# tpoisonooo/how-to-optimize-gemm

Measured on NVIDIA H100. Metric: SGEMM GFLOP/s (square N=4096 point of the 256..4096 sweep), higher is better.
Workload: dtype f16x2(scaled split-f32)

## Files before the change

### how-to-optimize-gemm_b200/csrc/capi.cu

```cuda
#include "../../include/b200gemm.h"

#include <cuda.h>
#include <cuda_runtime.h>
#include <stdio.h>
#include <stdlib.h>
#include <string.h>

#include <atomic>
#include <mutex>
#include <vector>

#include "gemm_ffma.cuh"
#include "gemm_generic.cuh"
#include "gemm_mxf4.cuh"
#include "gemm_tc.cuh"

using namespace b200;

namespace {

std::atomic<unsigned long long> g_launches{0};
int g_split_tail = 1;

struct KernelTimer {
  static constexpr int CAP = 1024;
  bool on = false;
  int n = 0;
  cudaEvent_t ev[CAP][2] = {};
  void begin(cudaStream_t st) {
    if (!on || n >= CAP) return;
    if (!ev[n][0]) { cudaEventCreate(&ev[n][0]); cudaEventCreate(&ev[n][1]); }
    cudaEventRecord(ev[n][0], st);
  }
  void end(cudaStream_t st) {
    if (!on || n >= CAP) return;
    cudaEventRecord(ev[n][1], st);
    n++;
  }
} g_ktimer;
std::atomic<int> g_default_f32_mode{-1};
thread_local const char* t_last_kernel = "none";
struct Schedule { int tiles = 0, split = 0, full_tiles = 0, ctas = 0; };
thread_local Schedule t_last_schedule;
int g_dbg_b_lbo = 0, g_dbg_b_sbo = 0;

struct Call {
  cudaStream_t st = nullptr;
  int acc = 0;
  int axpby = 0;
  float alpha = 1.f, beta = 0.f;
  const void* bias = nullptr;
  int act = -1;
  int sm_reserve = 0;
  bool epi() const { return act >= 0; }
};

constexpr int kFlagSlots = 16;
struct Scratch { void* p = nullptr; size_t bytes = 0; };
struct HostPipe {
  bool ready = false;
  cudaStream_t h2d = nullptr, comp = nullptr, d2h = nullptr;
  cudaEvent_t in[8] = {}, done[8] = {};
  cudaError_t init() {
    if (ready) return cudaSuccess;
    cudaError_t e;
    if ((e = cudaStreamCreateWithFlags(&h2d, cudaStreamNonBlocking)) != cudaSuccess) return e;
    if ((e = cudaStreamCreateWithFlags(&comp, cudaStreamNonBlocking)) != cudaSuccess) return e;
    if ((e = cudaStreamCreateWithFlags(&d2h, cudaStreamNonBlocking)) != cudaSuccess) return e;
    for (int i = 0; i < 8; i++) {
      if ((e = cudaEventCreateWithFlags(&in[i], cudaEventDisableTiming)) != cudaSuccess) return e;
      if ((e = cudaEventCreateWithFlags(&done[i], cudaEventDisableTiming)) != cudaSuccess) return e;
    }
    ready = true;
    return cudaSuccess;
  }
};
struct DevCtx {
  int ok = 0;
  int sms = 0;
  int dev = -1;
  int* flags = nullptr;
  std::mutex flag_mu;
  unsigned flag_slot = 0;
  struct FlagUser {
    cudaStream_t st = nullptr;
    cudaEvent_t ev = nullptr;
    bool used = false;
  } flag_user[kFlagSlots];
  std::mutex ws_mu;
  Scratch ws;
  cudaEvent_t ws_event = nullptr;
  cudaStream_t ws_stream = nullptr;
  bool ws_busy = false;
  struct MaxBuf {
    unsigned slot = 0;
    float* buf = nullptr;
    size_t cap = 0;
    int dirty[2] = {0, 0};
  } cmax, amax;
  cudaStream_t aux = nullptr;
  cudaEvent_t aux_fork = nullptr, aux_join = nullptr;
  std::mutex host_mu;
  Scratch scr[4];
  HostPipe pipe;
  std::vector<const void*> attr_done;
};
constexpr int kMaxDevices = 64;
DevCtx g_ctx[kMaxDevices];
std::mutex g_mu;

typedef CUresult (*EncodeTiledFn)(CUtensorMap*, CUtensorMapDataType, cuuint32_t, void*,
                                  const cuuint64_t*, const cuuint64_t*, const cuuint32_t*,
                                  const cuuint32_t*, CUtensorMapInterleave, CUtensorMapSwizzle,
                                  CUtensorMapL2promotion, CUtensorMapFloatOOBfill);
EncodeTiledFn g_encode = nullptr;

thread_local DevCtx* t_ctx = nullptr;
thread_local int t_bound_dev = -1;

int ensure_device() {
  int dev = -1;
  if (cudaGetDevice(&dev) != cudaSuccess || dev < 0 || dev >= kMaxDevices) { cudaGetLastError(); t_ctx = nullptr; return B200_ERR_NO_DEVICE; }
  if (t_bound_dev != dev) {
    if (cudaSetDevice(dev) != cudaSuccess) { cudaGetLastError(); t_ctx = nullptr; return B200_ERR_NO_DEVICE; }
    t_bound_dev = dev;
  }
  DevCtx* c = &g_ctx[dev];
  t_ctx = c;
  if (c->ok == 1) return 0;
  std::lock_guard<std::mutex> lk(g_mu);
  if (c->ok == 1) return 0;
  cudaDeviceProp prop;
  if (cudaGetDeviceProperties(&prop, dev) != cudaSuccess) { cudaGetLastError(); c->ok = -1; return B200_ERR_NO_DEVICE; }
  if (prop.major != 9) { c->ok = -1; return B200_ERR_NO_DEVICE; }
  if (!g_encode) {
    void* fn = nullptr;
    cudaDriverEntryPointQueryResult qres;
    if (cudaGetDriverEntryPoint("cuTensorMapEncodeTiled", &fn, cudaEnableDefault, &qres) != cudaSuccess ||
        qres != cudaDriverEntryPointSuccess || !fn) {
      cudaGetLastError();
      c->ok = -1;
      return B200_ERR_NO_DEVICE;
    }
    g_encode = reinterpret_cast<EncodeTiledFn>(fn);
  }
  if (!c->flags) {
    if (cudaMalloc(&c->flags, kFlagSlots * 1024 * sizeof(int)) != cudaSuccess ||
        cudaMemset(c->flags, 0, kFlagSlots * 1024 * sizeof(int)) != cudaSuccess) {
      cudaGetLastError(); c->flags = nullptr; c->ok = -1; return B200_ERR_NO_DEVICE;
    }
  }
  if (!c->ws_event && cudaEventCreateWithFlags(&c->ws_event, cudaEventDisableTiming) != cudaSuccess) {
    cudaGetLastError(); c->ok = -1; return B200_ERR_NO_DEVICE;
  }
  for (auto& u : c->flag_user)
    if (!u.ev && cudaEventCreateWithFlags(&u.ev, cudaEventDisableTiming) != cudaSuccess) {
      cudaGetLastError(); u.ev = nullptr; c->ok = -1; return B200_ERR_NO_DEVICE;
    }
  c->dev = dev;
  c->sms = prop.multiProcessorCount;
  c->ok = 1;
  return 0;
}

template <typename Kern>
int ensure_smem_attr(Kern kern, int bytes) {
  const void* key = reinterpret_cast<const void*>(kern);
  {
    std::lock_guard<std::mutex> lk(g_mu);
    for (const void* k : t_ctx->attr_done) if (k == key) return 0;
  }
  cudaError_t e = cudaFuncSetAttribute(kern, cudaFuncAttributeMaxDynamicSharedMemorySize, bytes);
  if (e != cudaSuccess) { cudaGetLastError(); return (int)e; }
  std::lock_guard<std::mutex> lk(g_mu);
  t_ctx->attr_done.push_back(key);
  return 0;
}

struct MapKey {
  const void* ptr; int dtype; unsigned long long d0, d1, ld_bytes; unsigned b0, b1; int swz; int dev;
  unsigned long long d2, d2_bytes;
  bool operator==(const MapKey& o) const {
    return ptr == o.ptr && dtype == o.dtype && d0 == o.d0 && d1 == o.d1 && ld_bytes == o.ld_bytes &&
           b0 == o.b0 && b1 == o.b1 && swz == o.swz && dev == o.dev && d2 == o.d2 && d2_bytes == o.d2_bytes;
  }
};
struct MapEntry { MapKey key; CUtensorMap map; };
std::vector<MapEntry> g_maps;
size_t g_map_next = 0;
constexpr size_t kMapCache = 64;

int get_map(CUtensorMap* out, const void* ptr, CUtensorMapDataType dt, int elem_bytes,
            unsigned long long inner, unsigned long long rows, unsigned long long ld_bytes,
            unsigned box_inner, unsigned box_rows, int swizzle ,
            unsigned long long entries = 0, unsigned long long entry_bytes = 0) {
  MapKey key{ptr, (int)dt, inner, rows, ld_bytes, box_inner, box_rows, swizzle, t_ctx->dev, entries, entry_bytes};
  std::lock_guard<std::mutex> lk(g_mu);
  for (auto& e : g_maps)
    if (e.key == key) { *out = e.map; return 0; }
  cuuint64_t dims[3] = {inner, rows, entries};
  cuuint64_t strides[2] = {ld_bytes, entry_bytes};
  cuuint32_t box[3] = {box_inner, box_rows, 1};
  cuuint32_t estr[3] = {1, 1, 1};
  CUtensorMap m;
  CUresult r = g_encode(&m, dt, entries ? 3 : 2, const_cast<void*>(ptr), dims, strides, box, estr,
                        CU_TENSOR_MAP_INTERLEAVE_NONE,
                        swizzle == 1 ? CU_TENSOR_MAP_SWIZZLE_128B
                        : swizzle == 2 ? CU_TENSOR_MAP_SWIZZLE_128B_ATOM_32B
                        : swizzle == 3 ? CU_TENSOR_MAP_SWIZZLE_64B : CU_TENSOR_MAP_SWIZZLE_NONE,
                        CU_TENSOR_MAP_L2_PROMOTION_L2_256B, CU_TENSOR_MAP_FLOAT_OOB_FILL_NONE);
  (void)elem_bytes;
  if (r != CUDA_SUCCESS) return B200_ERR_TENSORMAP;
  if (g_maps.size() < kMapCache) g_maps.push_back({key, m});
  else { g_maps[g_map_next] = {key, m}; g_map_next = (g_map_next + 1) % kMapCache; }
  *out = m;
  return 0;
}

inline bool aligned16(const void* p) { return (reinterpret_cast<uintptr_t>(p) & 15) == 0; }

int check_args(int m, int n, int k, const void* A, int lda, const void* B, int ldb, const void* C, int ldc,
               int op_a = B200_OP_N, int op_b = B200_OP_N) {
  if ((op_a != B200_OP_N && op_a != B200_OP_T) || (op_b != B200_OP_N && op_b != B200_OP_T)) return B200_ERR_BAD_ARG;
  if (m < 0 || n < 0 || k < 0) return B200_ERR_BAD_ARG;
  if (m == 0 || n == 0) return 1;
  if (!C || ldc < n) return B200_ERR_BAD_ARG;
  if (k > 0 && (!A || !B || lda < (op_a ? m : k) || ldb < (op_b ? k : n))) return B200_ERR_BAD_ARG;
  return 0;
}

int last_launch_status() {
  cudaError_t e = cudaPeekAtLastError();
  if (e != cudaSuccess) { cudaGetLastError(); return (int)e; }
  return 0;
}

int g_pdl = 1;
int g_prepass_fork = 1;
template <typename... KArgs, typename... Args>
cudaError_t launch_pdl(void (*kern)(KArgs...), dim3 grid, dim3 block, size_t smem, cudaStream_t st, int cluster, Args&&... args) {
  cudaLaunchConfig_t cfg = {};
  cfg.gridDim = grid; cfg.blockDim = block; cfg.dynamicSmemBytes = smem; cfg.stream = st;
  cudaLaunchAttribute at[2];
  int n = 0;
  if (cluster > 1) {
    at[n].id = cudaLaunchAttributeClusterDimension;
    at[n].val.clusterDim.x = cluster; at[n].val.clusterDim.y = 1; at[n].val.clusterDim.z = 1;
    n++;
  }
  if (g_pdl) {
    at[n].id = cudaLaunchAttributeProgrammaticStreamSerialization;
    at[n].val.programmaticStreamSerializationAllowed = 1;
    n++;
  }
  cfg.attrs = at; cfg.numAttrs = n;
  return cudaLaunchKernelEx(&cfg, kern, std::forward<Args>(args)...);
}

constexpr long long kMaxGridY = 65535;
inline unsigned grid_y(long long blocks) { return (unsigned)(blocks < kMaxGridY ? blocks : kMaxGridY); }

template <typename T>
int launch_zero(int m, int n, T* C, int ldc, cudaStream_t st) {
  dim3 grid((n + 255) / 256, m < 4096 ? m : 4096);
  fill_zero_kernel<T><<<grid, 256, 0, st>>>(m, n, C, ldc);
  g_launches++;
  t_last_kernel = "fill_zero";
  return last_launch_status();
}

template <typename InT, typename OutT>
int launch_generic(int op_a, int op_b, int m, int n, int k, const void* A, int lda, const void* B, int ldb, void* C,
                   int ldc, const char* name, const Call& c) {
  const long long mblocks = (m + 63LL) / 64;
  dim3 grid((n + 63) / 64, grid_y(mblocks));
  const long long a_rs = op_a ? 1 : lda, a_cs = op_a ? lda : 1, b_rs = op_b ? 1 : ldb, b_cs = op_b ? ldb : 1;
  auto kern = mblocks > kMaxGridY ? gemm_generic_kernel<InT, OutT, true> : gemm_generic_kernel<InT, OutT>;
  kern<<<grid, 256, 0, c.st>>>(m, n, k, static_cast<const InT*>(A), a_rs, a_cs, static_cast<const InT*>(B), b_rs, b_cs,
                               static_cast<OutT*>(C), ldc, c.acc, nullptr, nullptr, c.axpby, c.alpha, c.beta,
                               static_cast<const InT*>(c.bias), c.act);
  g_launches++;
  t_last_kernel = name;
  return last_launch_status();
}

int launch_generic_requant(int m, int n, int k, const int8_t* A, int lda, const int8_t* B, int ldb, int8_t* C,
                           int ldc, const float* scales, const float* bias, cudaStream_t st) {
  const long long mblocks = (m + 63LL) / 64;
  dim3 grid((n + 63) / 64, grid_y(mblocks));
  auto kern = mblocks > kMaxGridY ? gemm_generic_kernel<int8_t, int8_t, true> : gemm_generic_kernel<int8_t, int8_t>;
  kern<<<grid, 256, 0, st>>>(m, n, k, A, lda, 1, B, ldb, 1, C, ldc, 0, scales, bias, 0, 1.f, 0.f, nullptr, -1);
  g_launches++;
  t_last_kernel = "generic_s8_requant_64x64";
  return last_launch_status();
}

int take_flag_slot(cudaStream_t st, int** flags, DevCtx::FlagUser** user) {
  DevCtx* c = t_ctx;
  const unsigned slot = c->flag_slot++ % kFlagSlots;
  *flags = c->flags + slot * 1024;
  *user = nullptr;
  cudaStreamCaptureStatus cs = cudaStreamCaptureStatusNone;
  if (cudaStreamIsCapturing(st, &cs) != cudaSuccess) { cudaGetLastError(); cs = cudaStreamCaptureStatusActive; }
  DevCtx::FlagUser* u = &c->flag_user[slot];
  cudaError_t e;
  if (cs == cudaStreamCaptureStatusNone) {
    if (u->used && (u->st != st || st == cudaStreamPerThread) && (e = cudaStreamWaitEvent(st, u->ev, 0)) != cudaSuccess) {
      cudaGetLastError();
      return (int)e;
    }
    *user = u;
// ... 278 lines not shown
}

inline long long pitch16(int cols, int elem) { return (((long long)cols * elem + 15) & ~15LL) / elem; }
inline size_t round1024(size_t b) { return (b + 1023) & ~(size_t)1023; }
size_t kmajor_ws_bytes(int op_a, int op_b, int m, int n, int k, int elem) {
  const size_t b = op_b ? 0 : (size_t)n * pitch16(k, elem) * elem;
  const size_t a = op_a ? (size_t)m * pitch16(k, elem) * elem : 0;
  return a ? round1024(b) + a : b;
}

template <typename E>
int stage_kmajor(int op_a, int op_b, int m, int n, int k, const void*& A, long long& lda, const void*& B, long long& ldb,
                 uint8_t* ws, cudaStream_t st, bool copy_a = false, bool copy_b = false) {
  const long long kp = pitch16(k, sizeof(E));
  if (!op_b) {
    E* d = reinterpret_cast<E*>(ws);
    if (copy_b) {
      const cudaError_t e = cudaMemcpy2DAsync(d, kp * sizeof(E), B, ldb * sizeof(E), (size_t)k * sizeof(E), n,
                                              cudaMemcpyDeviceToDevice, st);
      if (e != cudaSuccess) { cudaGetLastError(); return (int)e; }
    } else if (int rc = launch_transpose<E>(static_cast<const E*>(B), ldb, k, n, d, kp, st)) {
      return rc;
    }
    B = d; ldb = kp;
  }
  if (op_a) {
    E* d = reinterpret_cast<E*>(ws + (op_b ? 0 : round1024((size_t)n * kp * sizeof(E))));
    if (copy_a) {
      const cudaError_t e = cudaMemcpy2DAsync(d, kp * sizeof(E), A, lda * sizeof(E), (size_t)k * sizeof(E), m,
                                              cudaMemcpyDeviceToDevice, st);
      if (e != cudaSuccess) { cudaGetLastError(); return (int)e; }
    } else if (int rc = launch_transpose<E>(static_cast<const E*>(A), lda, k, m, d, kp, st)) {
      return rc;
    }
    A = d; lda = kp;
  }
  return 0;
}

template <int KIND, int BN, int STAGES, typename OutT>
int launch_tc_kmajor(int op_a, int op_b, int m, int n, int k, const void* A, long long lda, const void* B, long long ldb,
                     void* C, int ldc, const char* name, const Call& c, const float* row_max = nullptr,
                     const float* col_max = nullptr) {
  if (!op_a && op_b) return launch_tc<KIND, BN, STAGES, OutT>(m, n, k, A, lda, m, 0, B, ldb, n, 0, C, ldc, name, c, 0, row_max, col_max);
  using E = typename std::conditional<KIND == KIND_TF32, float, uint8_t>::type;
  WsLease ws(kmajor_ws_bytes(op_a, op_b, m, n, k, sizeof(E)), c.st);
  if (ws.rc) return ws.rc;
  if (int rc = stage_kmajor<E>(op_a, op_b, m, n, k, A, lda, B, ldb, ws.base(), c.st)) return rc;
  return launch_tc<KIND, BN, STAGES, OutT>(m, n, k, A, lda, m, 0, B, ldb, n, 0, C, ldc, name, c, 0, row_max, col_max);
}

const char* const kNamesTf32[3] = {"tc_tf32_128x256", "tc_tf32_128x192", "tc_tf32_128x128"};
int tc_tf32(int op_a, int op_b, int m, int n, int k, const void* A, int lda, const void* B, int ldb, void* C, int ldc,
            const Call& c) {
  return with_width(m, n, [&](auto W) {
    using Wd = decltype(W);
    return launch_tc_kmajor<KIND_TF32, Wd::BN, Wd::STAGES, float>(op_a, op_b, m, n, k, A, lda, B, ldb, C, ldc,
                                                                kNamesTf32[Wd::idx], c);
  });
}
int tc_s8(int op_a, int op_b, int m, int n, int k, const void* A, int lda, const void* B, int ldb, void* C, int ldc,
          const Call& c) {
  return with_width<false>(m, n, [&](auto W) {
    using Wd = decltype(W);
    return launch_tc_kmajor<KIND_I8, Wd::BN, Wd::STAGES, int32_t>(op_a, op_b, m, n, k, A, lda, B, ldb, C, ldc,
                                                                Wd::BN == 256 ? "tc_s8_128x256" : "tc_s8_128x128", c);
  });
}
int tc_s8_requant(int m, int n, int k, const void* A, int lda, const void* B, int ldb, void* C, int ldc,
                  const float* scales, const float* bias, const Call& c) {
  return with_width<false>(m, n, [&](auto W) {
    using Wd = decltype(W);
    return launch_tc_kmajor<KIND_I8, Wd::BN, Wd::STAGES, s8_out>(
        B200_OP_N, B200_OP_N, m, n, k, A, lda, B, ldb, C, ldc,
        Wd::BN == 256 ? "tc_s8_requant_128x256" : "tc_s8_requant_128x128", c, scales, bias);
  });
}

inline long long plane_pitch(int cols) { return ((long long)cols + 7) & ~7LL; }
inline int b_plane_rows(int k) { return (k + 31) & ~31; }

template <int NP>
int launch_split(const SplitJob& ja, const SplitJob& jb, int jobs, cudaStream_t st) {
  const long long wide = jobs == 2 && jb.dld > ja.dld ? jb.dld : ja.dld;
  const int tall = jobs == 2 && jb.plane_rows > ja.plane_rows ? jb.plane_rows : ja.plane_rows;
  const int gx = (int)((wide + 2047) / 2048);
  int gy = (t_ctx->sms * 8 + jobs * gx - 1) / (jobs * gx);
  if (gy > (tall + 1) / 2) gy = (tall + 1) / 2;
  if (gy < 1) gy = 1;
  launch_pdl(split_planes_kernel<NP>, dim3(gx, gy, jobs), dim3(256), 0, st, 1, ja, jb);
  g_launches += 1;
  return last_launch_status();
}

struct PlaneGeom {
  int rows, cols, plane_rows;
  long long pitch;
  size_t bytes(int np) const { return (size_t)np * plane_rows * pitch * 2; }
};
inline PlaneGeom plane_geom(bool k_along_rows, int rows, int cols) {
  return PlaneGeom{rows, cols, k_along_rows ? b_plane_rows(rows) : rows, plane_pitch(cols)};
}
inline PlaneGeom geom_a(int op_a, int m, int k) { return op_a ? plane_geom(true, k, m) : plane_geom(false, m, k); }
inline PlaneGeom geom_b(int op_b, int k, int n) { return op_b ? plane_geom(false, n, k) : plane_geom(true, k, n); }

size_t split_ws_bytes(int np, int op_a, int op_b, int m, int n, int k, bool prepB = false) {
  const size_t a = round1024(geom_a(op_a, m, k).bytes(np));
  return prepB ? a : a + geom_b(op_b, k, n).bytes(np);
}

KernelNames kNamesBf16x3 = TC_NAMES("tc_bf16x3"), kNamesBf16x2 = TC_NAMES("tc_bf16x2"), kNamesF16x2 = TC_NAMES("tc_f16x2");

template <int NP>
int gemm_f32_split(int op_a, int op_b, int m, int n, int k, const float* A, int lda, const float* B, int ldb, float* C,
                   int ldc, const uint16_t* prepB, const Call& c) {
  const PlaneGeom ga = geom_a(op_a, m, k), gb = geom_b(op_b, k, n);
  WsLease ws(split_ws_bytes(NP, op_a, op_b, m, n, k, prepB != nullptr), c.st);
  if (ws.rc) return ws.rc;
  uint16_t* pA = reinterpret_cast<uint16_t*>(ws.base());
  const uint16_t* pB = prepB ? prepB : reinterpret_cast<uint16_t*>(ws.base() + round1024(ga.bytes(NP)));
  const SplitJob ja{A, lda, ga.rows, ga.cols, pA, ga.pitch, ga.plane_rows},
                 jb{B, ldb, gb.rows, gb.cols, const_cast<uint16_t*>(pB), gb.pitch, gb.plane_rows};
  if (int rc = launch_split<NP>(ja, jb, prepB ? 1 : 2, c.st)) return rc;
  using Prod = typename std::conditional<NP == 3, ProdX3, ProdX2>::type;
  return with_layout(op_a, op_b, [&](auto L) {
    using Lay = decltype(L);
    return launch_tc<KIND_F16, 128, NP == 3 ? 4 : 6, float, Prod, 64, Lay::AL, Lay::BL>(
        m, n, k, pA, ga.pitch, NP * ga.plane_rows, ga.plane_rows, pB, gb.pitch, NP * gb.plane_rows, gb.plane_rows, C, ldc,
        (NP == 3 ? kNamesBf16x3 : kNamesBf16x2)[Lay::idx][2], c, g_split_chunk_k[NP == 3 ? 0 : 1]);
  });
}

struct F16Operand {
  const uint16_t* planes;
  long long pitch;
  int plane_rows;
  const float* maxv;
};

int launch_f16_split_rows(const float* A, long long lda, int rows, int cols, float* rmax, uint16_t* planes,
                          long long pitch, int plane_rows, cudaStream_t st) {
  int blocks = (plane_rows + 7) / 8;
  const int cap = t_ctx->sms * 16;
  if (blocks > cap) blocks = cap;
  if (blocks < 1) blocks = 1;
  if (cols <= 1024) launch_pdl(split_f16_rows_kernel<4>, dim3(blocks), dim3(256), 0, st, 1, A, (long long)lda, rows, cols, rmax, planes, pitch, plane_rows);
  else if (cols <= 2048) launch_pdl(split_f16_rows_kernel<8>, dim3(blocks), dim3(256), 0, st, 1, A, (long long)lda, rows, cols, rmax, planes, pitch, plane_rows);
  else if (cols <= 4096) launch_pdl(split_f16_rows_kernel<16>, dim3(blocks), dim3(256), 0, st, 1, A, (long long)lda, rows, cols, rmax, planes, pitch, plane_rows);
  else launch_pdl(split_f16_rows_kernel<0>, dim3(blocks), dim3(256), 0, st, 1, A, (long long)lda, rows, cols, rmax, planes, pitch, plane_rows);
  g_launches++;
  return last_launch_status();
}

int launch_f16_split_cols(const float* B, long long ldb, int rows, int cols, float* cmax, uint16_t* planes,
                          long long pitch, int plane_rows, float* zero_buf, int zero_n, cudaStream_t st) {
  const cudaError_t e1 = launch_pdl(col_absmax_kernel, dim3((cols + 1023) / 1024, grid_y((rows + 15LL) / 16)), dim3(256), 0,
                                    st, 1, B, (long long)ldb, rows, cols, reinterpret_cast<unsigned int*>(cmax));
  const int gx = (int)((pitch + 2047) / 2048);
  int gy = (t_ctx->sms * 8 + gx - 1) / gx;
  if (gy > (plane_rows + 1) / 2) gy = (plane_rows + 1) / 2;
  if (gy < 1) gy = 1;
  if (zero_buf && zero_n > gx * 2048) {
    cudaMemsetAsync(zero_buf, 0, (size_t)zero_n * 4, st);
    zero_buf = nullptr;
  }
  const cudaError_t e2 = launch_pdl(split_f16_cols_kernel, dim3(gx, gy), dim3(256), 0, st, 1, B, (long long)ldb, rows, cols, (const float*)cmax, planes, pitch, plane_rows, zero_buf, zero_n);
  g_launches += 2;
  if (e1 != cudaSuccess || e2 != cudaSuccess) { cudaGetLastError(); return (int)(e1 != cudaSuccess ? e1 : e2); }
  return last_launch_status();
}

int gemm_f16x2_core(int op_a, int op_b, int m, int n, int k, const F16Operand& a, const F16Operand& b, float* C, int ldc,
                    const Call& c) {
  constexpr int NP = 2;
  return with_layout(op_a, op_b, [&](auto L) {
    using Lay = decltype(L);
    return launch_tc<KIND_FP16, 128, 6, float, ProdX2, 64, Lay::AL, Lay::BL>(
        m, n, k, a.planes, a.pitch, NP * a.plane_rows, a.plane_rows, b.planes, b.pitch, NP * b.plane_rows, b.plane_rows, C,
        ldc, kNamesF16x2[Lay::idx][2], c, g_split_chunk_k[2], a.maxv, b.maxv);
  });
}

int cmax_reserve(DevCtx::MaxBuf& mb, int n, float** cur, float** other, int* other_dirty) {
  if (mb.cap < (size_t)n) {
    size_t cap = mb.cap ? 2 * mb.cap : 16384;
    if (cap < (size_t)n) cap = (size_t)n;
    if (mb.buf) { cudaDeviceSynchronize(); cudaFree(mb.buf); }
    mb.buf = nullptr; mb.cap = 0;
    cudaError_t e = cudaMalloc(&mb.buf, 2 * cap * sizeof(float));
    if (e == cudaSuccess) e = cudaMemset(mb.buf, 0, 2 * cap * sizeof(float));
    if (e != cudaSuccess) { cudaGetLastError(); return (int)e; }
    mb.cap = cap;
    mb.dirty[0] = mb.dirty[1] = 0;
  }
  const unsigned slot = mb.slot++ & 1u;
  *cur = mb.buf + slot * mb.cap;
  *other = mb.buf + (slot ^ 1u) * mb.cap;
  *other_dirty = mb.dirty[slot ^ 1u];
  mb.dirty[slot ^ 1u] = 0;
  mb.dirty[slot] = n;
  return 0;
}

struct F16Ws {
  PlaneGeom ga, gb;
  size_t a_off, r_off, rb_off, total;
};
F16Ws f16x2_ws(int op_a, int op_b, int m, int n, int k, bool prepA, bool prepB) {
  F16Ws w{geom_a(op_a, m, k), geom_b(op_b, k, n)};
  w.a_off = round1024(prepA ? 0 : w.ga.bytes(2));
  w.r_off = round1024(w.a_off + (prepB ? 0 : w.gb.bytes(2)));
  const size_t ra = prepA || op_a ? 0 : (size_t)m * 4;
  w.rb_off = round1024(w.r_off + ra);
  w.total = prepB || !op_b ? w.r_off + ra : w.rb_off + (size_t)n * 4;
  return w;
}

int gemm_f32_split_f16(int op_a, int op_b, int m, int n, int k, const float* A, int lda, const float* B, int ldb, float* C,
                       int ldc, const F16Operand* prepA, const F16Operand* prepB, const Call& c) {
  if (prepA && prepB) return gemm_f16x2_core(B200_OP_N, B200_OP_N, m, n, k, *prepA, *prepB, C, ldc, c);
  const F16Ws w = f16x2_ws(op_a, op_b, m, n, k, prepA != nullptr, prepB != nullptr);
  const PlaneGeom &ga = w.ga, &gb = w.gb;
  WsLease ws(w.total, c.st);
  if (ws.rc) return ws.rc;
  uint8_t* base = ws.base();
  F16Operand oa, ob;
  DevCtx* dc = t_ctx;
  const bool fork = !prepA && !prepB && g_prepass_fork && (double)m * k + (double)k * n >= 4.0e6;
  cudaStream_t sb = c.st;
  if (fork) {
    if (!dc->aux) {
      if (cudaStreamCreateWithFlags(&dc->aux, cudaStreamNonBlocking) != cudaSuccess ||
          cudaEventCreateWithFlags(&dc->aux_fork, cudaEventDisableTiming) != cudaSuccess ||
          cudaEventCreateWithFlags(&dc->aux_join, cudaEventDisableTiming) != cudaSuccess) { cudaGetLastError(); return B200_ERR_NO_DEVICE; }
    }
    cudaEventRecord(dc->aux_fork, c.st);
    cudaStreamWaitEvent(dc->aux, dc->aux_fork, 0);
    sb = dc->aux;
  }
  if (prepB) ob = *prepB;
  else if (op_b) {
    uint16_t* pB = reinterpret_cast<uint16_t*>(base + w.a_off);
    float* bmax = reinterpret_cast<float*>(base + w.rb_off);
    if (int rc = launch_f16_split_rows(B, ldb, n, k, bmax, pB, gb.pitch, gb.plane_rows, sb)) return rc;
    ob = F16Operand{pB, gb.pitch, gb.plane_rows, bmax};
  } else {
    uint16_t* pB = reinterpret_cast<uint16_t*>(base + w.a_off);
    float *cmax, *other;
    int other_dirty;
    if (int rc = cmax_reserve(dc->cmax, n, &cmax, &other, &other_dirty)) return rc;
    if (int rc = launch_f16_split_cols(B, ldb, k, n, cmax, pB, gb.pitch, gb.plane_rows, other, other_dirty, sb)) return rc;
    ob = F16Operand{pB, gb.pitch, gb.plane_rows, cmax};
  }
  if (prepA) oa = *prepA;
  else if (op_a) {
    uint16_t* pA = reinterpret_cast<uint16_t*>(base);
    float *amax, *other;
    int other_dirty;
    if (int rc = cmax_reserve(dc->amax, m, &amax, &other, &other_dirty)) return rc;
    if (int rc = launch_f16_split_cols(A, lda, k, m, amax, pA, ga.pitch, ga.plane_rows, other, other_dirty, c.st)) return rc;
    oa = F16Operand{pA, ga.pitch, ga.plane_rows, amax};
  } else {
    uint16_t* pA = reinterpret_cast<uint16_t*>(base);
    float* rmax = reinterpret_cast<float*>(base + w.r_off);
    if (int rc = launch_f16_split_rows(A, lda, m, k, rmax, pA, ga.pitch, ga.plane_rows, c.st)) return rc;
    oa = F16Operand{pA, ga.pitch, ga.plane_rows, rmax};
  }
  if (fork) {
    cudaEventRecord(dc->aux_join, dc->aux);
    cudaStreamWaitEvent(c.st, dc->aux_join, 0);
  }
  return gemm_f16x2_core(op_a, op_b, m, n, k, oa, ob, C, ldc, c);
}

template <class Cfg, class Kern>
int launch_ffma(Kern kern, int ctas_per_sm, const char* name, int m, int n, int k, const float* A, int lda,
                const float* B, int ldb, float* C, int ldc, const Call& c) {
  CUtensorMap tmA, tmB;
  int rc = get_map(&tmA, A, CU_TENSOR_MAP_DATA_TYPE_FLOAT32, 4, k, m, (unsigned long long)lda * 4, Cfg::BK, Cfg::BM, 1);
  if (rc) return rc;
  rc = get_map(&tmB, B, CU_TENSOR_MAP_DATA_TYPE_FLOAT32, 4, n, k, (unsigned long long)ldb * 4, Cfg::BN, Cfg::BK, 0);
  if (rc) return rc;
  FfmaParams p;
  p.C = C; p.ldc = ldc; p.M = m; p.N = n; p.K = k;
  p.vec_ok = aligned16(C) && (ldc % 4) == 0;
  p.accumulate = c.acc;
  p.axpby = c.axpby; p.alpha = c.alpha; p.beta = c.beta;
  p.tiles_m = (m + Cfg::BM - 1) / Cfg::BM;
  p.tiles_n = (n + Cfg::BN - 1) / Cfg::BN;
  p.group_m = 8;
  const int tiles = p.tiles_m * p.tiles_n, slots = ctas_per_sm * t_ctx->sms;
  const int rem = tiles % slots;
  const bool halves = g_ffma_halves && rem > 0 && 2 * rem <= slots;
  p.full_tiles = halves ? tiles - rem : tiles;
  const int ctas = p.full_tiles + 2 * (tiles - p.full_tiles);
  if (int arc = ensure_smem_attr(kern, Cfg::SMEM_BYTES)) return arc;
  g_ktimer.begin(c.st);
  kern<<<ctas, Cfg::THREADS, Cfg::SMEM_BYTES, c.st>>>(tmA, tmB, p);
  g_ktimer.end(c.st);
  g_launches++;
  t_last_kernel = name;
  return last_launch_status();
}

size_t strict_ws_bytes(int op_a, int op_b, int m, int n, int k) {
  const size_t a = op_a ? (size_t)m * pitch16(k, 4) * 4 : 0, b = op_b ? (size_t)k * pitch16(n, 4) * 4 : 0;
  return a && b ? round1024(a) + b : a + b;
}
// ... 1265 lines not shown
```

### how-to-optimize-gemm_b200/csrc/gemm_tc.cuh

```cuda
#pragma once
#include <cuda_fp16.h>
#include <string.h>
#include <type_traits>

#include "ptx.cuh"
#include "wgmma.cuh"

namespace b200 {

enum Layout { LAYOUT_K = 0, LAYOUT_MN = 1 };

template <int KIND> struct KindTraits;
template <> struct KindTraits<KIND_F16>  { static constexpr int ELEM = 2; static constexpr int B_LAYOUT = LAYOUT_MN; };
template <> struct KindTraits<KIND_FP16> { static constexpr int ELEM = 2; static constexpr int B_LAYOUT = LAYOUT_MN; };
template <> struct KindTraits<KIND_TF32> { static constexpr int ELEM = 4; static constexpr int B_LAYOUT = LAYOUT_K; };
template <> struct KindTraits<KIND_I8>   { static constexpr int ELEM = 1; static constexpr int B_LAYOUT = LAYOUT_K; };
template <> struct KindTraits<KIND_E4M3> { static constexpr int ELEM = 1; static constexpr int B_LAYOUT = LAYOUT_K; };
template <> struct KindTraits<KIND_E4M3E5M2> { static constexpr int ELEM = 1; static constexpr int B_LAYOUT = LAYOUT_K; };
template <> struct KindTraits<KIND_E5M2E4M3> { static constexpr int ELEM = 1; static constexpr int B_LAYOUT = LAYOUT_K; };

struct ProdSingle {
  static constexpr int N = 1, NPA = 1, NPB = 1;
  __host__ __device__ static constexpr int ia(int) { return 0; }
  __host__ __device__ static constexpr int ib(int) { return 0; }
// ... 1505 lines not shown
      for (int c = lane * 8; c < dld; c += 256) {
        *reinterpret_cast<uint4*>(d1 + c) = make_uint4(0, 0, 0, 0);
        *reinterpret_cast<uint4*>(d2 + c) = make_uint4(0, 0, 0, 0);
      }
      continue;
    }
    const float* s = src + (long long)r * ld;
    float mx = 0.f;
    if constexpr (VPL > 0) {
      float x[VPL][8];
#pragma unroll
      for (int j = 0; j < VPL; j++) {
        const int c = (j * 32 + lane) * 8;
#pragma unroll
        for (int e = 0; e < 8; e++) x[j][e] = 0.f;
        if (c < cols) load8(s, c, cols, vec, x[j]);
#pragma unroll
        for (int e = 0; e < 8; e++) mx = fmaxf(mx, fabsf(x[j][e]));
      }
#pragma unroll
      for (int o = 16; o > 0; o >>= 1) mx = fmaxf(mx, __shfl_xor_sync(0xffffffffu, mx, o));
      if (lane == 0) rmax[r] = mx;
      const int ex = -pow2_exp(mx);
#pragma unroll
      for (int j = 0; j < VPL; j++) {
        const int c = (j * 32 + lane) * 8;
        if (c < dld) {
#pragma unroll
          for (int e = 0; e < 8; e++) x[j][e] = scale_pow2(x[j][e], ex);
          uint4 h1, h2;
          split_f16x8(x[j], h1, h2);
          *reinterpret_cast<uint4*>(d1 + c) = h1;
          *reinterpret_cast<uint4*>(d2 + c) = h2;
        }
      }
    } else {
      for (int c0 = lane * 8; c0 < cols; c0 += 1024) {
        float x[4][8];
#pragma unroll
        for (int u = 0; u < 4; u++) {
          const int c = c0 + u * 256;
#pragma unroll
          for (int e = 0; e < 8; e++) x[u][e] = 0.f;
          if (c < cols) load8(s, c, cols, vec, x[u]);
#pragma unroll
          for (int e = 0; e < 8; e++) mx = fmaxf(mx, fabsf(x[u][e]));
        }
      }
#pragma unroll
      for (int o = 16; o > 0; o >>= 1) mx = fmaxf(mx, __shfl_xor_sync(0xffffffffu, mx, o));
      if (lane == 0) rmax[r] = mx;
      const int ex = -pow2_exp(mx);
      for (int c0 = lane * 8; c0 < dld; c0 += 512) {
        float x[2][8];
#pragma unroll
        for (int u = 0; u < 2; u++) {
          const int c = c0 + u * 256;
#pragma unroll
          for (int e = 0; e < 8; e++) x[u][e] = 0.f;
          if (c < cols) load8(s, c, cols, vec, x[u]);
        }
#pragma unroll
        for (int u = 0; u < 2; u++) {
          const int c = c0 + u * 256;
          if (c < dld) {
#pragma unroll
            for (int e = 0; e < 8; e++) x[u][e] = scale_pow2(x[u][e], ex);
            uint4 h1, h2;
            split_f16x8(x[u], h1, h2);
            *reinterpret_cast<uint4*>(d1 + c) = h1;
            *reinterpret_cast<uint4*>(d2 + c) = h2;
          }
        }
      }
    }
  }
}

__global__ void __launch_bounds__(256) col_absmax_kernel(const float* __restrict__ src, long long ld, int rows,
                                                         int cols, unsigned int* __restrict__ out) {
  constexpr int ROWS = 16;
  griddep_launch();
  griddep_wait();
  const int c = blockIdx.x * 1024 + threadIdx.x * 4;
  if (c >= cols) return;
  const int rblocks = (int)(((long long)rows + ROWS - 1) / ROWS);
  const bool vec = (ld & 3) == 0 && (reinterpret_cast<uintptr_t>(src) & 15) == 0 && c + 4 <= cols;
  float4 mx = make_float4(0.f, 0.f, 0.f, 0.f);
  for (int rb = blockIdx.y; rb < rblocks; rb += gridDim.y) {
    const int r0 = rb * ROWS, r1 = min(r0 + ROWS, rows);
    if (vec) {
#pragma unroll 16
      for (int r = r0; r < r1; r++) {
        const float4 v = __ldg(reinterpret_cast<const float4*>(src + (long long)r * ld + c));
        mx.x = fmaxf(mx.x, fabsf(v.x)); mx.y = fmaxf(mx.y, fabsf(v.y));
        mx.z = fmaxf(mx.z, fabsf(v.z)); mx.w = fmaxf(mx.w, fabsf(v.w));
      }
    } else {
      for (int r = r0; r < r1; r++) {
        const float* s = src + (long long)r * ld + c;
        mx.x = fmaxf(mx.x, fabsf(s[0]));
        if (c + 1 < cols) mx.y = fmaxf(mx.y, fabsf(s[1]));
        if (c + 2 < cols) mx.z = fmaxf(mx.z, fabsf(s[2]));
        if (c + 3 < cols) mx.w = fmaxf(mx.w, fabsf(s[3]));
      }
    }
  }
  const float m4[4] = {mx.x, mx.y, mx.z, mx.w};
#pragma unroll
  for (int e = 0; e < 4; e++)
    if (c + e < cols && __float_as_uint(m4[e]) > __ldcg(out + c + e)) atomicMax(out + c + e, __float_as_uint(m4[e]));
}

__global__ void __launch_bounds__(256) split_f16_cols_kernel(const float* __restrict__ src, long long ld, int rows,
                                                             int cols, const float* __restrict__ cmax,
                                                             uint16_t* __restrict__ dst, long long dld, int plane_rows,
                                                             float* __restrict__ zero_buf, int zero_n) {
  griddep_launch();
  griddep_wait();
  const int c = (int)(blockIdx.x * 256 + threadIdx.x) * 8;
  if (blockIdx.y == 0 && zero_buf != nullptr) {
#pragma unroll
    for (int e = 0; e < 8; e++)
      if (c + e < zero_n) zero_buf[c + e] = 0.f;
  }
  if (c >= dld) return;
  const bool vec = (ld & 3) == 0 && (reinterpret_cast<uintptr_t>(src) & 15) == 0;
  int ex[8];
#pragma unroll
  for (int e = 0; e < 8; e++) ex[e] = c + e < cols ? -pow2_exp(__ldg(cmax + c + e)) : 0;
  for (int r0 = blockIdx.y * 2; r0 < plane_rows; r0 += gridDim.y * 2) {
    float x[2][8];
#pragma unroll
    for (int u = 0; u < 2; u++) {
      const int r = r0 + u;
#pragma unroll
      for (int e = 0; e < 8; e++) x[u][e] = 0.f;
      if (r < rows) load8(src + (long long)r * ld, c, cols, vec, x[u]);
    }
#pragma unroll
    for (int u = 0; u < 2; u++) {
      const int r = r0 + u;
      if (r >= plane_rows) break;
#pragma unroll
      for (int e = 0; e < 8; e++) x[u][e] = scale_pow2(x[u][e], ex[e]);
      uint4 h1, h2;
      split_f16x8(x[u], h1, h2);
      *reinterpret_cast<uint4*>(dst + (long long)r * dld + c) = h1;
      *reinterpret_cast<uint4*>(dst + ((long long)plane_rows + r) * dld + c) = h2;
    }
  }
}

}
```

### how-to-optimize-gemm_b200/csrc/ptx.cuh

```cuda
#pragma once
#include <cuda.h>
#include <cuda_runtime.h>
#include <math.h>
#include <stdint.h>

namespace b200 {

__device__ __forceinline__ uint32_t smem_u32(const void* p) {
  return static_cast<uint32_t>(__cvta_generic_to_shared(p));
}

__device__ __forceinline__ void mbar_init(uint32_t bar, uint32_t count) {
  asm volatile("mbarrier.init.shared::cta.b64 [%0], %1;" ::"r"(bar), "r"(count) : "memory");
}
__device__ __forceinline__ void fence_barrier_init() {
  asm volatile("fence.mbarrier_init.release.cluster;" ::: "memory");
}
__device__ __forceinline__ void fence_proxy_async() {
  asm volatile("fence.proxy.async.shared::cta;" ::: "memory");
}
__device__ __forceinline__ void mbar_arrive_expect_tx(uint32_t bar, uint32_t bytes) {
  asm volatile("mbarrier.arrive.expect_tx.shared::cta.b64 _, [%0], %1;" ::"r"(bar), "r"(bytes)
               : "memory");
}
__device__ __forceinline__ void mbar_arrive(uint32_t bar) {
  asm volatile("mbarrier.arrive.shared::cta.b64 _, [%0];" ::"r"(bar) : "memory");
}
__device__ __forceinline__ bool mbar_try_wait(uint32_t bar, uint32_t parity) {
  uint32_t ok;
  asm volatile(
      "{\n\t.reg .pred p;\n\t"
      "mbarrier.try_wait.parity.shared::cta.b64 p, [%1], %2;\n\t"
      "selp.u32 %0, 1, 0, p;\n\t}"
      : "=r"(ok)
      : "r"(bar), "r"(parity)
      : "memory");
  return ok != 0;
}
__device__ __forceinline__ void mbar_wait(uint32_t bar, uint32_t parity) {
  if (mbar_try_wait(bar, parity)) return;
  const long long t0 = clock64();
  while (!mbar_try_wait(bar, parity)) {
    if (clock64() - t0 > 4000000000LL) { asm volatile("trap;"); }
  }
}

__device__ __forceinline__ void tma_prefetch_desc(const CUtensorMap* m) {
  asm volatile("prefetch.tensormap [%0];" ::"l"(reinterpret_cast<uint64_t>(m)) : "memory");
}
__device__ __forceinline__ void tma_load_2d(uint32_t dst_smem, const CUtensorMap* m, uint32_t bar,
                                            int c0, int c1) {
  asm volatile(
      "cp.async.bulk.tensor.2d.shared::cluster.global.tile.mbarrier::complete_tx::bytes "
      "[%0], [%1, {%3, %4}], [%2];"
      ::"r"(dst_smem), "l"(reinterpret_cast<uint64_t>(m)), "r"(bar), "r"(c0), "r"(c1)
      : "memory");
}
__device__ __forceinline__ void tma_load_3d(uint32_t dst_smem, const CUtensorMap* m, uint32_t bar,
                                            int c0, int c1, int c2) {
  asm volatile(
      "cp.async.bulk.tensor.3d.shared::cluster.global.tile.mbarrier::complete_tx::bytes "
      "[%0], [%1, {%3, %4, %5}], [%2];"
      ::"r"(dst_smem), "l"(reinterpret_cast<uint64_t>(m)), "r"(bar), "r"(c0), "r"(c1), "r"(c2)
      : "memory");
}
__device__ __forceinline__ void tma_load_2d_hint(uint32_t dst_smem, const CUtensorMap* m,
                                                 uint32_t bar, int c0, int c1, uint64_t policy) {
  asm volatile(
      "cp.async.bulk.tensor.2d.shared::cluster.global.tile.mbarrier::complete_tx::bytes"
      ".L2::cache_hint [%0], [%1, {%3, %4}], [%2], %5;"
      ::"r"(dst_smem), "l"(reinterpret_cast<uint64_t>(m)), "r"(bar), "r"(c0), "r"(c1), "l"(policy)
      : "memory");
}

enum MmaKind { KIND_F16 = 0 , KIND_TF32 = 1, KIND_I8 = 2, KIND_FP16 = 3 ,
               KIND_E4M3 = 4 , KIND_E4M3E5M2 = 5 , KIND_E5M2E4M3 = 6  };
enum Swz { SWZ_128B = 1, SWZ_64B = 2 };

__device__ __forceinline__ uint64_t make_sdesc(uint32_t smem_addr, uint32_t lbo_bytes, uint32_t sbo_bytes, uint32_t swz) {
  uint64_t d = 0;
  d |= (uint64_t)((smem_addr & 0x3FFFF) >> 4);
  d |= (uint64_t)((lbo_bytes >> 4) & 0x3FFF) << 16;
  d |= (uint64_t)((sbo_bytes >> 4) & 0x3FFF) << 32;
  d |= (uint64_t)swz << 62;
  return d;
}

__device__ __forceinline__ int32_t requant_s8(int32_t acc, float scale, float bias, bool has_bias) {
  float f = __fmul_rn(__int2float_rn(acc), scale);
  if (has_bias) f = __fadd_rn(f, bias);
  const float g = fminf(fmaxf(f, -200.0f), 200.0f);
  const float magic = 12582912.0f;
  float r = __fadd_rn(__fadd_rn(g, magic), -magic);
  if (fabsf(__fadd_rn(g, -r)) == 0.5f && fabsf(r) < fabsf(g)) r = __fadd_rn(r, copysignf(1.0f, g));
  r = fminf(fmaxf(r, -128.0f), 127.0f);
  const int32_t q = __float_as_int(__fadd_rn(r, magic)) - 0x4B400000;
  return f != f ? 0 : q;
}

enum EpiAct { ACT_NONE = 0, ACT_RELU = 1, ACT_GELU = 2, ACT_GELU_TANH = 3 };
template <int ACT>
__device__ __forceinline__ float epi_act(float t) {
  if constexpr (ACT == ACT_RELU) {
    return t < 0.f ? 0.f : t;
  } else if constexpr (ACT == ACT_GELU) {
    const float g = __fmul_rn(__fmul_rn(0.5f, t), erfcf(__fmul_rn(-0.707106781186547524f, t)));
    return t == -INFINITY ? -0.f : g;
  } else if constexpr (ACT == ACT_GELU_TANH) {
    const float u = __fmul_rn(0.797884560802865356f, __fmaf_rn(__fmul_rn(0.044715f, t), __fmul_rn(t, t), t));
    const float g = __fmul_rn(__fmul_rn(0.5f, t), __fadd_rn(1.f, tanhf(u)));
    return t == -INFINITY ? -0.f : g;
  } else {
    return t;
  }
}

template <int N> __device__ __forceinline__ void setmaxnreg_inc() { asm volatile("setmaxnreg.inc.sync.aligned.u32 %0;" ::"n"(N)); }
template <int N> __device__ __forceinline__ void setmaxnreg_dec() { asm volatile("setmaxnreg.dec.sync.aligned.u32 %0;" ::"n"(N)); }

__device__ __forceinline__ void griddep_launch() { asm volatile("griddepcontrol.launch_dependents;" ::: "memory"); }
__device__ __forceinline__ void griddep_wait() { asm volatile("griddepcontrol.wait;" ::: "memory"); }

__device__ __forceinline__ bool elect_one() {
  uint32_t pred;
  asm volatile("{\n\t.reg .pred p;\n\telect.sync _|p, 0xffffffff;\n\tselp.b32 %0, 1, 0, p;\n\t}" : "=r"(pred));
  return pred != 0;
}

constexpr int kMaxGroups = 1024;

__device__ __forceinline__ void group_table(const int* __restrict__ offs, int groups, int total_m, int rows, int* end,
                                            int* block) {
  for (int i = threadIdx.x; i < groups; i += blockDim.x) end[i + 1] = offs[i];
  __syncthreads();
  if (threadIdx.x < 32) {
    const int lane = threadIdx.x;
    int run_end = 0, run_blocks = 0;
    for (int base = 0; base < groups; base += 32) {
      const int g = base + lane;
      int e = max(g < groups ? end[g + 1] : 0, run_end);
#pragma unroll
      for (int d = 1; d < 32; d <<= 1) {
        const int o = __shfl_up_sync(0xffffffffu, e, d);
        if (lane >= d) e = max(e, o);
      }
      e = min(e, total_m);
      int prev = __shfl_up_sync(0xffffffffu, e, 1);
      if (lane == 0) prev = run_end;
      int b = (e - prev) / rows + ((e - prev) % rows != 0);
#pragma unroll
      for (int d = 1; d < 32; d <<= 1) {
        const int o = __shfl_up_sync(0xffffffffu, b, d);
        if (lane >= d) b += o;
      }
      if (g < groups) { end[g + 1] = e; block[g + 1] = run_blocks + b; }
      run_end = __shfl_sync(0xffffffffu, e, 31);
      run_blocks += __shfl_sync(0xffffffffu, b, 31);
    }
    if (lane == 0) { end[0] = 0; block[0] = 0; }
  }
  __syncthreads();
}

__device__ __forceinline__ int group_of(const int* block, int groups, int q) {
  int lo = 0, hi = groups - 1;
  while (lo < hi) {
    const int mid = (lo + hi + 1) >> 1;
    if (block[mid] <= q) lo = mid;
    else hi = mid - 1;
  }
  return lo;
}

}
```

Baseline: 187,800.

## Fuse column absmax and f16 split of B into one cluster strip kernel

Replaces the two-kernel path for B (column absmax pass, then split pass) with one kernel launched in 8-CTA clusters. Each cluster owns a 32-column strip and each CTA stages its share of rows in shared memory via cp.async. The CTAs reduce the per-column max across the cluster through distributed shared memory, then scale and split from shared memory. This reads B from global memory once instead of twice and saves a launch, at the cost of heavy shared memory use, cluster barriers and a size-gated fallback.

```diff
diff --git a/how-to-optimize-gemm_b200/csrc/capi.cu b/how-to-optimize-gemm_b200/csrc/capi.cu
--- a/how-to-optimize-gemm_b200/csrc/capi.cu
+++ b/how-to-optimize-gemm_b200/csrc/capi.cu
@@ -99,6 +99,7 @@
     int dirty[2] = {0, 0};
   } cmax, amax;
   cudaStream_t aux = nullptr;
+  int strip_rows = 0;
   cudaEvent_t aux_fork = nullptr, aux_join = nullptr;
   std::mutex host_mu;
   Scratch scr[4];
@@ -157,6 +158,9 @@
     if (!u.ev && cudaEventCreateWithFlags(&u.ev, cudaEventDisableTiming) != cudaSuccess) {
       cudaGetLastError(); u.ev = nullptr; c->ok = -1; return B200_ERR_NO_DEVICE;
     }
+  cudaFuncAttributes fa;
+  if (cudaFuncGetAttributes(&fa, split_f16_strip_kernel) != cudaSuccess) { cudaGetLastError(); c->ok = -1; return B200_ERR_NO_DEVICE; }
+  c->strip_rows = (int)((prop.sharedMemPerBlockOptin - fa.sharedSizeBytes) / (kStripW * sizeof(float)));
   c->dev = dev;
   c->sms = prop.multiProcessorCount;
   c->ok = 1;
@@ -741,8 +745,24 @@
   return last_launch_status();
 }
 
+constexpr int kStripCluster = 8, kStripWave = 3;
 int launch_f16_split_cols(const float* B, long long ldb, int rows, int cols, float* cmax, uint16_t* planes,
                           long long pitch, int plane_rows, float* zero_buf, int zero_n, cudaStream_t st) {
+  const int rp = (plane_rows + kStripCluster - 1) / kStripCluster;
+  const long long strips = (pitch + kStripW - 1) / kStripW;
+  if (rp <= t_ctx->strip_rows && strips * kStripCluster >= (long long)kStripWave * t_ctx->sms) {
+    if (int arc = ensure_smem_attr(split_f16_strip_kernel, t_ctx->strip_rows * kStripW * (int)sizeof(float))) return arc;
+    const cudaError_t e = launch_pdl(split_f16_strip_kernel, dim3((unsigned)(strips * kStripCluster)), dim3(256),
+                                     (size_t)rp * kStripW * sizeof(float), st, kStripCluster, B, (long long)ldb, rows,
+                                     cols, cmax, planes, pitch, plane_rows, rp, zero_buf, zero_n);
+    g_launches++;
+    if (e != cudaSuccess) {
+      cudaGetLastError();
+      if (zero_buf) cudaMemsetAsync(zero_buf, 0, (size_t)zero_n * 4, st);
+      return (int)e;
+    }
+    return last_launch_status();
+  }
   const cudaError_t e1 = launch_pdl(col_absmax_kernel, dim3((cols + 1023) / 1024, grid_y((rows + 15LL) / 16)), dim3(256), 0,
                                     st, 1, B, (long long)ldb, rows, cols, reinterpret_cast<unsigned int*>(cmax));
   const int gx = (int)((pitch + 2047) / 2048);
diff --git a/how-to-optimize-gemm_b200/csrc/gemm_tc.cuh b/how-to-optimize-gemm_b200/csrc/gemm_tc.cuh
--- a/how-to-optimize-gemm_b200/csrc/gemm_tc.cuh
+++ b/how-to-optimize-gemm_b200/csrc/gemm_tc.cuh
@@ -1681,4 +1681,92 @@
   }
 }
 
-}
+constexpr int kStripW = 32;
+__global__ void __launch_bounds__(256) split_f16_strip_kernel(const float* __restrict__ src, long long ld, int rows,
+                                                              int cols, float* __restrict__ cmax,
+                                                              uint16_t* __restrict__ dst, long long dld, int plane_rows,
+                                                              int rp, float* __restrict__ zero_buf, int zero_n) {
+  extern __shared__ __align__(16) float strip[];
+  __shared__ float red[8][kStripW];
+  __shared__ float part[kStripW], full[kStripW];
+  griddep_launch();
+  griddep_wait();
+  const int t = threadIdx.x;
+  if (zero_buf != nullptr)
+    for (long long i = (long long)blockIdx.x * 256 + t; i < zero_n; i += (long long)gridDim.x * 256) zero_buf[i] = 0.f;
+  const uint32_t rank = cluster_ctarank(), ncta = cluster_nctarank();
+  const int c0 = (int)(blockIdx.x / ncta) * kStripW;
+  const int r0 = (int)rank * rp;
+  const int np = max(min(r0 + rp, plane_rows) - r0, 0);
+  const int nl = max(min(r0 + rp, rows) - r0, 0);
+  {
+    const bool vec = (ld & 3) == 0 && (reinterpret_cast<uintptr_t>(src) & 15) == 0;
+    const int q = t & 7, c = c0 + 4 * q;
+    const int valid = min(max(cols - c, 0), 4);
+    for (int r = t >> 3; r < nl; r += 32) {
+      const float* s = src + (long long)(r0 + r) * ld + c;
+      const uint32_t d = smem_u32(strip + r * kStripW + 4 * q);
+      if (vec) {
+        asm volatile("cp.async.cg.shared.global [%0], [%1], 16, %2;" ::"r"(d), "l"(valid ? s : src), "r"(valid * 4) : "memory");
+      } else {
+#pragma unroll
+        for (int e = 0; e < 4; e++)
+          asm volatile("cp.async.ca.shared.global [%0], [%1], 4, %2;" ::"r"(d + 4 * e), "l"(e < valid ? s + e : src),
+                       "r"(e < valid ? 4 : 0) : "memory");
+      }
+    }
+    asm volatile("cp.async.wait_all;" ::: "memory");
+    __syncthreads();
+  }
+  {
+    const int j = t & (kStripW - 1), g = t >> 5;
+    float m = 0.f;
+#pragma unroll 8
+    for (int r = g; r < nl; r += 8) m = fmaxf(m, fabsf(strip[r * kStripW + j]));
+    red[g][j] = m;
+    __syncthreads();
+    if (t < kStripW) {
+#pragma unroll
+      for (int k = 1; k < 8; k++) m = fmaxf(m, red[k][t]);
+      part[t] = m;
+    }
+  }
+  cluster_arrive();
+  cluster_wait();
+  if (t < kStripW) {
+    float m = 0.f;
+    for (uint32_t k = 0; k < ncta; k++) m = fmaxf(m, ld_shared_cluster(&part[t], k));
+    full[t] = m;
+    if (rank == 0 && c0 + t < cols) cmax[c0 + t] = m;
+  }
+  cluster_arrive();
+  __syncthreads();
+  const int q = t & 3, c = c0 + 8 * q;
+  if (c < dld) {
+    int ex[8];
+#pragma unroll
+    for (int e = 0; e < 8; e++) ex[e] = c + e < cols ? -pow2_exp(full[8 * q + e]) : 0;
+    for (int r = t >> 2; r < np; r += 64) {
+      float x[8];
+      if (r < nl) {
+        const float4 v0 = *reinterpret_cast<const float4*>(strip + r * kStripW + 8 * q);
+        const float4 v1 = *reinterpret_cast<const float4*>(strip + r * kStripW + 8 * q + 4);
+        x[0] = v0.x; x[1] = v0.y; x[2] = v0.z; x[3] = v0.w;
+        x[4] = v1.x; x[5] = v1.y; x[6] = v1.z; x[7] = v1.w;
+      } else {
+#pragma unroll
+        for (int e = 0; e < 8; e++) x[e] = 0.f;
+      }
+#pragma unroll
+      for (int e = 0; e < 8; e++) x[e] = scale_pow2(x[e], ex[e]);
+      uint4 h1, h2;
+      split_f16x8(x, h1, h2);
+      const long long pr = r0 + r;
+      *reinterpret_cast<uint4*>(dst + pr * dld + c) = h1;
+      *reinterpret_cast<uint4*>(dst + ((long long)plane_rows + pr) * dld + c) = h2;
+    }
+  }
+  cluster_wait();
+}
+
+}
diff --git a/how-to-optimize-gemm_b200/csrc/ptx.cuh b/how-to-optimize-gemm_b200/csrc/ptx.cuh
--- a/how-to-optimize-gemm_b200/csrc/ptx.cuh
+++ b/how-to-optimize-gemm_b200/csrc/ptx.cuh
@@ -121,6 +121,18 @@
 __device__ __forceinline__ void griddep_launch() { asm volatile("griddepcontrol.launch_dependents;" ::: "memory"); }
 __device__ __forceinline__ void griddep_wait() { asm volatile("griddepcontrol.wait;" ::: "memory"); }
 
+__device__ __forceinline__ uint32_t cluster_ctarank() { uint32_t r; asm volatile("mov.u32 %0, %%cluster_ctarank;" : "=r"(r)); return r; }
+__device__ __forceinline__ uint32_t cluster_nctarank() { uint32_t r; asm volatile("mov.u32 %0, %%cluster_nctarank;" : "=r"(r)); return r; }
+__device__ __forceinline__ void cluster_arrive() { asm volatile("barrier.cluster.arrive.release.aligned;" ::: "memory"); }
+__device__ __forceinline__ void cluster_wait() { asm volatile("barrier.cluster.wait.acquire.aligned;" ::: "memory"); }
+__device__ __forceinline__ float ld_shared_cluster(const void* p, uint32_t rank) {
+  uint32_t remote;
+  float v;
+  asm volatile("mapa.shared::cluster.u32 %0, %1, %2;" : "=r"(remote) : "r"(smem_u32(p)), "r"(rank));
+  asm volatile("ld.shared::cluster.f32 %0, [%1];" : "=f"(v) : "r"(remote) : "memory");
+  return v;
+}
+
 __device__ __forceinline__ bool elect_one() {
   uint32_t pred;
   asm volatile("{\n\t.reg .pred p;\n\telect.sync _|p, 0xffffffff;\n\tselp.b32 %0, 1, 0, p;\n\t}" : "=r"(pred));
```

New measurement: 193,300, median of 6. +2.9%, better.
